# snayfach/MicrobeCensus

Measured on AMD Instinct MI355X. Metric: reads/sec searched vs marker DB + AGS abs-error, 150 bp @ 1/2/4/8 GPU, higher is better.
Workload: dtype u8/int32

## Files before the change

microbecensus_amd/csrc/k_translate_seg.h:

```cpp
#pragma once
#include "mc_hip_common.h"

#define MC_TS_THREADS 64
#define MC_TS_WAVES (MC_TS_THREADS / 64)
#define MC_TS_READS (MC_TS_THREADS / 6)
#define MC_TS_NLNF(FP) ((FP) + 2 > 24 ? (FP) + 2 : 24)
#define MC_TS_STRIDE(FP) (((((FP) + 76 + 3) >> 2) | 1) << 2)
#define MC_TS_STAGE(L) ((((MC_TS_READS * (L)) > MC_TS_WAVES * 1488 ? (MC_TS_READS * (L)) : MC_TS_WAVES * 1488) + 15) & ~15)

struct McSegWaveLds { unsigned long long best[64]; uint32_t pre[66]; uint32_t pre2[66]; uint32_t bq[64]; uint16_t off[64]; uint8_t n[64]; };
static_assert(sizeof(McHsp) == 48 && sizeof(McGapTask) % 4 == 0, "k_eval_seeds copies its staging buffers as 16- and 4-byte words");
static_assert(sizeof(McSegWaveLds) == 1488, "MC_TS_STAGE reserves 1488 bytes per wave");
#ifdef MC_EXP_TIMING
__device__ unsigned long long g_ts_acc[12], g_ts_cnt[12];
#define MC_TS_TICK(k) do { const unsigned long long now_ = __builtin_readcyclecounter(); if (lane == 0) { ts_acc_[tcat_] += now_ - tlast_; ts_acc_[12 + tcat_] += 1; } tlast_ = now_; tcat_ = (k); } while (0)
#define MC_TS_BEGIN(k) __shared__ unsigned long long ts_acc_[24]; if (lane < 24) ts_acc_[lane] = 0; mc_wave_sync(); unsigned long long tlast_ = __builtin_readcyclecounter(); int tcat_ = (k)
#define MC_TS_PARAMS , unsigned long long &tlast_, int &tcat_, unsigned long long *ts_acc_
#define MC_TS_ARGS , tlast_, tcat_, ts_acc_
#define MC_TS_END do { mc_wave_sync(); if (lane < 12) { atomicAdd(&g_ts_acc[lane], ts_acc_[lane]); atomicAdd(&g_ts_cnt[lane], ts_acc_[12 + lane]); } } while (0)
#else
#define MC_TS_TICK(k) do { } while (0)
#define MC_TS_BEGIN(k) do { } while (0)
#define MC_TS_PARAMS
#define MC_TS_ARGS
#define MC_TS_END do { } while (0)
#endif
#define MC_SEG_KEY_ONE 0xBFF0000000000000ull

__device__ __forceinline__ unsigned long long mc_seg_key(double x)
{
    const unsigned long long u = (unsigned long long)__double_as_longlong(x);
    return (u >> 63) ? ~u : (u | 0x8000000000000000ull);
}

__device__ __forceinline__ void mc_seg_wave(const double *lnf, const int32_t *fx, const uint64_t *__restrict__ segtab, uint8_t *prot, int n, bool act, const McSegWS ws, McSegWaveLds *WL,
                                         const uint8_t *lds0, int lane MC_TS_PARAMS)
{
    const int W = (n <= 11) ? 8 : 12;
    MC_TS_TICK(0);
    enum { POP = 0, SCAN = 1, WAIT = 2, DONE = 3 };
    int st = (act && W <= n) ? POP : DONE;
    McBits192 Flo, Fhi, lo, nhi, mk;
    mc_bits_clear(Flo); mc_bits_clear(Fhi); mc_bits_clear(lo); mc_bits_clear(nhi); mc_bits_clear(mk);
    if (st != DONE) {
        mc_seg_window_flags_rg(fx, prot, n, W, Flo, Fhi);
        if (!(Flo.a | Flo.b | Flo.c)) st = DONE;
    }
    int sp = 1, base = 0, m = 0, i = 0, lowlim = 0, loi = 0, hii = 0;
    bool any = false;
    if (st != DONE) { ws.stk[0] = 0; ws.stk[1] = (int16_t)n; }
    const unsigned long long ltmask = (1ull << lane) - 1;
    for (;;) {
        MC_TS_TICK(1);
        while (st == POP || st == SCAN) {
            if (st == POP) {
                if (sp == 0) { st = DONE; break; }
                sp--;
                base = ws.stk[2 * sp]; m = ws.stk[2 * sp + 1];
                if (W > m) continue;
                lo = mc_seg_flags_of(Flo, base, m, W);
                i = mc_bits_next(lo, 0);
                if (i >= m) continue;
                nhi = mc_bits_andnot(mc_bits_low(m), mc_seg_flags_of(Fhi, base, m, W));
                lowlim = 0; st = SCAN;
            }
            loi = mc_bits_prev(nhi, i) + 1; if (loi < lowlim) loi = lowlim;
            hii = mc_bits_next(nhi, i) - 1; if (hii > m - 1) hii = m - 1;
            st = WAIT;
        }
        const unsigned long long req = __ballot(st == WAIT);
        MC_TS_TICK(2);
        if (req == 0) break;
        const int nreq = __popcll(req);
        const int myr = __popcll(req & ltmask);
        const int myn = hii - loi + 1;
        if (st == WAIT) {
            WL->off[myr] = (uint16_t)((prot + base + loi) - lds0);
            WL->n[myr] = (uint8_t)myn;
            WL->best[myr] = MC_SEG_KEY_ONE; WL->bq[myr] = 0xFFFFFFFFu;
        }
        mc_wave_sync();
#define MC_SEG_CJ(j, sh) (((((j) >> (sh)) * (((j) >> (sh)) + 1)) << (sh)) / 2 + ((j) & ((1 << (sh)) - 1)) * (((j) >> (sh)) + 1))
        int sh0 = 3, sh1 = 3;
        {
            int K = 0, j0 = 0;
            if (lane < nreq) { const int nn = WL->n[lane], minlen = (nn - 100 > 1) ? nn - 100 : 1; K = nn - minlen; j0 = nn - 15 > 0 ? (nn - 15 < K ? nn - 15 : K) : 0; }
            uint32_t s0 = 0, s1 = 0;
#pragma unroll
            for (int sh = 2; sh >= 0; sh--) {
                const uint32_t c1 = (uint32_t)MC_SEG_CJ(j0, sh), c0 = (uint32_t)MC_SEG_CJ(K, sh) - c1;
                const uint32_t t0 = (uint32_t)__builtin_amdgcn_readlane((int)mc_wave_scan_add(c0), 63), t1 = (uint32_t)__builtin_amdgcn_readlane((int)mc_wave_scan_add(c1), 63);
                if (t0 <= 64) sh0 = sh;
                if (t1 <= 64) sh1 = sh;
            }
            {
                const uint32_t c1 = sh1 == 0 ? (uint32_t)MC_SEG_CJ(j0, 0) : sh1 == 1 ? (uint32_t)MC_SEG_CJ(j0, 1) : sh1 == 2 ? (uint32_t)MC_SEG_CJ(j0, 2) : (uint32_t)MC_SEG_CJ(j0, 3);
                const uint32_t cj0 = sh0 == 0 ? (uint32_t)MC_SEG_CJ(j0, 0) : sh0 == 1 ? (uint32_t)MC_SEG_CJ(j0, 1) : sh0 == 2 ? (uint32_t)MC_SEG_CJ(j0, 2) : (uint32_t)MC_SEG_CJ(j0, 3);
                const uint32_t ck = sh0 == 0 ? (uint32_t)MC_SEG_CJ(K, 0) : sh0 == 1 ? (uint32_t)MC_SEG_CJ(K, 1) : sh0 == 2 ? (uint32_t)MC_SEG_CJ(K, 2) : (uint32_t)MC_SEG_CJ(K, 3);
                s0 = mc_wave_scan_add(ck - cj0); s1 = mc_wave_scan_add(c1);
            }
            if (lane == 0) { WL->pre[0] = 0; WL->pre2[0] = 0; }
            WL->pre[lane + 1] = s0; WL->pre2[lane + 1] = s1;
        }
        mc_wave_sync();
        for (int cls = 0; cls < 2; cls++) {
        const uint32_t *pre = cls ? WL->pre2 : WL->pre;
        const uint32_t total = pre[nreq];
        const int sh = cls ? sh1 : sh0, R = 1 << sh;
        for (uint32_t p0 = 0; p0 < total; p0 += 64) {
            MC_TS_TICK(3 + cls);
            const uint32_t p = p0 + (uint32_t)lane;
            const bool ok = p < total;
            int r = 0;
            for (int stp = 32; stp > 0; stp >>= 1) { const int k = r + stp; if (k < nreq && p >= pre[k]) r = k; }
            if (!ok) r = 0;
            const int nn = WL->n[r];
            int x = (int)(p - pre[r]);
            if (cls == 0) { const int minlen = (nn - 100 > 1) ? nn - 100 : 1, K = nn - minlen, j0 = nn - 15 > 0 ? (nn - 15 < K ? nn - 15 : K) : 0; x += MC_SEG_CJ(j0, sh); }
            int A = (int)((sqrtf(1.0f + 8.0f * (float)x / (float)R) - 1.0f) * 0.5f);
            while ((((A + 1) * (A + 2)) << sh) / 2 <= x) A++;
            while (((A * (A + 1)) << sh) / 2 > x) A--;
            const int rem = x - ((A * (A + 1)) << sh) / 2, B = rem / (A + 1), run = rem - B * (A + 1);
            const int j = (A << sh) + B, wfirst = run << sh, wlast = (wfirst + R - 1 < j) ? wfirst + R - 1 : j;
            const uint8_t *s = lds0 + WL->off[r];
            const int len = nn - j;
            const uint32_t qbase = (uint32_t)(j * (j + 1) / 2);
            unsigned long long key = MC_SEG_KEY_ONE;
            uint32_t kq = 0xFFFFFFFFu;
            if (ok) {
                if (cls == 0) {
                    McRhState rg; rg.clo = 0; rg.chi = 0; rg.hist = 0;
                    for (int k = 0; k < len; k++) mc_rh_add(rg, s[wfirst + k]);
                    const int cnt = wlast - wfirst + 1;
                    uint64_t svs[8];
#pragma unroll
                    for (int t = 0; t < 8; t++) {
                        svs[t] = rg.hist | ((uint64_t)len << 60);
                        if (t + 1 < cnt) { mc_rh_remove(rg, s[wfirst + t]); mc_rh_add(rg, s[wfirst + t + len]); }
                    }
#pragma unroll
                    for (int t0 = 0; t0 < 8; t0 += 4) {
                        if (t0 && R <= 4) break;
                        ulonglong2 ea[4], eb[4];
#pragma unroll
                        for (int t = 0; t < 4; t++) {
                            uint32_t h1, h2;
                            mc_segtab_slots(svs[t0 + t], h1, h2);
                            const bool in = t0 + t < cnt;
                            ea[t] = ((const ulonglong2 *)segtab)[in ? h1 : 0u]; eb[t] = ((const ulonglong2 *)segtab)[in ? h2 : 0u];
                        }
#pragma unroll
                        for (int t = 0; t < 4; t++)
                            if (t0 + t < cnt) {
                                const unsigned long long pk = ea[t].x == svs[t0 + t] ? ea[t].y : eb[t].y;
                                if (pk < key) { key = pk; kq = qbase + (uint32_t)(wfirst + t0 + t); }
                            }
                    }
                } else {
                    mc_seg_comp_rg(s + wfirst, len, ws.comp);
                    mc_seg_state(ws.comp, ws.sv);
                    for (int w0 = wfirst;; w0++) {
                        const unsigned long long k2 = mc_seg_key(mc_seg_getprob(lnf, ws.sv, len));
                        if (k2 < key) { key = k2; kq = qbase + (uint32_t)w0; }
                        if (w0 == wlast) break;
                        mc_seg_shift(ws.comp, ws.sv, s[w0], s[w0 + len]);
                    }
                }
            }
            MC_TS_TICK(5);
            const bool cand = ok && key < MC_SEG_KEY_ONE;
            const unsigned long long old = WL->best[r];
            mc_wave_sync();
            if (cand) atomicMin(&WL->best[r], key);
            mc_wave_sync();
            const unsigned long long nb = WL->best[r];
            if (ok && nb != old) WL->bq[r] = 0xFFFFFFFFu;
            mc_wave_sync();
            if (cand && key == nb) atomicMin(&WL->bq[r], kq);
            mc_wave_sync();
        }
        }
#undef MC_SEG_CJ
        MC_TS_TICK(6);
        if (st == WAIT) {
            const uint32_t q = WL->bq[myr];
            int lend = 0, rend = myn - 1;
            if (q != 0xFFFFFFFFu) {
                int j = (int)((sqrtf((float)(8u * q + 1u)) - 1.0f) * 0.5f);
                while ((uint32_t)((j + 1) * (j + 2) / 2) <= q) j++;
                while ((uint32_t)(j * (j + 1) / 2) > q) j--;
                const int len = myn - j, w0 = (int)q - j * (j + 1) / 2;
                lend = w0; rend = len + w0 - 1;
            }
            const int leftend = loi + lend, rightend = hii - (myn - rend - 1);
            if (i < leftend) {
                const int l2 = loi, r2 = leftend - 1;
// ... 33 lines not shown
            w[k >> 2] |= ((a0 | a1 | a2) < 0 ? (uint32_t)MC_INV : aa) << (8 * (k & 3));
        }
        *(uint32_t *)(prot + i) = w[0];
        *(uint32_t *)(prot + i + 4) = w[1];
    }
    for (; i < n; i++) {
        const int a0 = mc_nt_code(p[s * (3 * i)], set, perm), a1 = mc_nt_code(p[s * (3 * i + 1)], set, perm), a2 = mc_nt_code(p[s * (3 * i + 2)], set, perm);
        const uint8_t aa = cod[(16 * a0 + 4 * a1 + a2) & 63];
        prot[i] = (a0 | a1 | a2) < 0 ? (uint8_t)MC_INV : aa;
    }
    return n;
}

template <bool STAGED>
__global__ void __attribute__((amdgpu_waves_per_eu(4, 4))) __launch_bounds__(MC_TS_THREADS) k_translate_seg(const McTables *__restrict__ T, const uint8_t *__restrict__ reads, int L,
                                                       int64_t nreads, uint8_t *__restrict__ frames, int FP, const uint64_t *__restrict__ segtab)
{
    extern __shared__ __attribute__((aligned(16))) uint8_t smem[];
    const int tid = threadIdx.x;
    const int64_t r0 = (int64_t)blockIdx.x * MC_TS_READS;
    const int nr = (int)((nreads - r0) < MC_TS_READS ? (nreads - r0) : MC_TS_READS);
    const int rbytes = nr * L;
    const int stride = MC_TS_STRIDE(FP);
    __shared__ int32_t fxs[64];
#ifdef MC_EXP_TIMING
    const int lane = mc_lane();
#endif
    MC_TS_BEGIN(8);
    uint8_t *sreads = smem;
    const int nlnf = MC_TS_NLNF(FP);
    double *lnf = (double *)(smem + (STAGED ? MC_TS_STAGE(L) : MC_TS_STAGE(0)));
    uint8_t *rows = (uint8_t *)(lnf + nlnf);
    __shared__ __attribute__((aligned(4))) uint8_t cod[64];
    if (tid < 64) fxs[tid] = T->seg_dout[tid];
    if (tid < 16) ((uint32_t *)cod)[tid] = ((const uint32_t *)T->codon)[tid];
    for (int i = tid; i < nlnf; i += MC_TS_THREADS) lnf[i] = T->lnfac[i];
    if (STAGED) {
        const uint8_t *src = reads + r0 * L;
        const int head = (int)((4 - ((uintptr_t)src & 3)) & 3), nhead = head < rbytes ? head : rbytes;
        if (tid < nhead) sreads[tid] = src[tid];
        const int nw = (rbytes - nhead) >> 2;
        if (nhead == 0) for (int i = tid; i < nw; i += MC_TS_THREADS) ((uint32_t *)sreads)[i] = ((const uint32_t *)src)[i];
        else for (int i = tid; i < nw; i += MC_TS_THREADS) { const uint32_t w = ((const uint32_t *)(src + nhead))[i]; uint8_t *d = sreads + nhead + 4 * i; d[0] = (uint8_t)w; d[1] = (uint8_t)(w >> 8); d[2] = (uint8_t)(w >> 16); d[3] = (uint8_t)(w >> 24); }
        for (int i = nhead + 4 * nw + tid; i < rbytes; i += MC_TS_THREADS) sreads[i] = src[i];
    }
    __syncthreads();
    MC_TS_TICK(9);
    const int lr = tid / 6, f = tid - lr * 6;
    uint8_t *prot = rows + (size_t)tid * stride;
    int n = 0;
    if (lr < nr) n = mc_translate_frame_lds(cod, STAGED ? sreads + lr * L : reads + (r0 + lr) * L, L, f, prot);
    __syncthreads();
    {
        McSegWS ws; ws.comp = prot + FP; ws.sv = prot + FP + 20; ws.stk = (int16_t *)(prot + FP + 44);
        mc_seg_wave(lnf, fxs, segtab, prot, n, lr < nr, ws, (McSegWaveLds *)smem + (tid >> 6), rows, mc_lane() MC_TS_ARGS);
        if (lr < nr) for (int i = n; i < FP; i++) prot[i] = MC_INV;
    }
    __syncthreads();
    {
        uint32_t *dst = (uint32_t *)(frames + r0 * 6 * FP);
        const int total = nr * 6 * FP / 4, fpw = FP / 4;
        for (int i = tid; i < total; i += MC_TS_THREADS) { const int row = i / fpw, col = i - row * fpw; dst[i] = *(const uint32_t *)(rows + (size_t)row * stride + 4 * col); }
    }
    MC_TS_TICK(0);
    MC_TS_END;
}
```

microbecensus_amd/csrc/mc_core.h:

```cpp
#pragma once
#include <stdint.h>

#if defined(__HIPCC__)
#include <hip/hip_runtime.h>
#define MC_HD __host__ __device__ __forceinline__
#define MC_HDN __host__ __device__
#else
#define MC_HD inline
#define MC_HDN inline
struct uint4 { uint32_t x, y, z, w; };
inline uint4 make_uint4(uint32_t x, uint32_t y, uint32_t z, uint32_t w) { uint4 v; v.x = x; v.y = y; v.z = z; v.w = w; return v; }
#endif

#define MC_NBUCKET 1000000
#define MC_INV 20
#define MC_INVGRP 10
#define MC_MAXAA 170
#define MC_SMAX 4096
#define MC_MAX_M8 500
#define MC_LNFAC_N 400

#define MC_GAP_OPEN 11
#define MC_GAP_EXT 1
#define MC_SEG_FXBITS 24
// ... 375 lines not shown
MC_HD void mc_segtab_slots(uint64_t k, uint32_t &h1, uint32_t &h2)
{
    const uint32_t lo = (uint32_t)k, hi = (uint32_t)(k >> 32);
    uint32_t x = (lo ^ (hi << 7) ^ (((hi >> 28) * 0x924000u) & 0x04444000u)) * 0xBA1BF32Fu;
    x ^= x >> 15;
    h1 = x >> (32 - MC_SEGTAB_LOG2);
    h2 = (x >> 6) & (MC_SEGTAB_SLOTS - 1);
}
MC_HD uint64_t mc_segtab_lookup(const uint64_t *tab, uint64_t hist, int len)
{
    const uint64_t k = hist | ((uint64_t)len << 60);
    uint32_t h1, h2;
    mc_segtab_slots(k, h1, h2);
    if (tab[2 * h1] == k) return tab[2 * h1 + 1];
    return tab[2 * h2] == k ? tab[2 * h2 + 1] : 0;
}

MC_HD void mc_seg_trim_rg(const double *lnfac, const uint8_t *s, int n, int *leftend, int *rightend)
{
    int lend = 0, rend = n - 1;
    double minprob = 1.0;
    McRgState st0; st0.clo = 0; st0.chi = 0; st0.sv = 0;
    for (int k = 0; k < n; k++) mc_rg_add(st0, s[k]);
    for (int len = n; len > 1; len--) {
        McRgState st = st0;
        for (int i = 0;; i++) {
            const double prob = mc_rg_getprob(lnfac, st.sv, len);
            if (prob < minprob) { minprob = prob; lend = i; rend = len + i - 1; }
            if (i + 1 + len > n) break;
            mc_rg_remove(st, s[i]); mc_rg_add(st, s[i + len]);
// ... 242 lines not shown
    int sp = 1;
    ws.stk[0] = 0; ws.stk[1] = (int16_t)n;
    bool any = false;
    while (sp > 0) {
        sp--;
        const int base = ws.stk[2 * sp], m = ws.stk[2 * sp + 1];
        const uint8_t *s = prot + base;
        if (W > m) continue;
        const McBits192 lo = mc_seg_flags_of(Flo, base, m, W), hi = mc_seg_flags_of(Fhi, base, m, W);
        const McBits192 nhi = mc_bits_andnot(mc_bits_low(m), hi);
        int lowlim = 0;
        for (int i = mc_bits_next(lo, 0); i < m; i = mc_bits_next(lo, i + 1)) {
            int loi = mc_bits_prev(nhi, i) + 1; if (loi < lowlim) loi = lowlim;
            int hii = mc_bits_next(nhi, i) - 1; if (hii > m - 1) hii = m - 1;
            int leftend = loi, rightend = hii;
            if (rightend - leftend + 1 <= 15) mc_seg_trim_rg(lnfac, s + leftend, rightend - leftend + 1, &leftend, &rightend);
            else mc_seg_trim_ws(lnfac, s + leftend, rightend - leftend + 1, &leftend, &rightend, ws);
            if (i < leftend) {
                const int lend = loi, rend = leftend - 1;
                if (sp < 8) { ws.stk[2 * sp] = (int16_t)(base + lend); ws.stk[2 * sp + 1] = (int16_t)(rend - lend + 1); sp++; }
            }
            mk = mc_bits_or(mk, mc_bits_range(base + leftend, base + rightend));
            any = true;
            i = (hii < rightend) ? hii : rightend;
            lowlim = i + 1;
        }
    }
    if (any) for (int i = 0; i < n; i++) if (mc_bits_test(mk, i)) prot[i] = MC_INV;
}

// ... 682 lines not shown
```

microbecensus_amd/csrc/mc_hip.hip:

```cpp
#include "mc_hip_common.h"
#include "k_translate_seg.h"
#include "k_enumerate.h"
#include "k_eval_seeds.h"
#include "k_gapped.h"
#include "k_order.h"
#include "k_finish.h"
#include "k_grid.h"
#include "k_simulate.h"
#include "k_community.h"
#include "k_varlen.h"
#include "k_bootstrap.h"

#include <map>

struct McCtx {
    hipStream_t stream = nullptr, side = nullptr, side2 = nullptr;
    hipEvent_t ev[8] = {}, ev_fork = nullptr, ev_join = nullptr, ev_join2 = nullptr;
    int64_t cap_reads = 0; int pool_len = 0;
    uint32_t cap_tasks = 0, cap_gaps = 0, cap_hsps = 0, cap_rows = 0;
    uint8_t *d_frames = nullptr, *d_frames_base = nullptr;
    unsigned long long *d_stats = nullptr;
    McSeedTask *d_tasks = nullptr; McGapTask *d_gaps = nullptr; McHsp *d_hsps = nullptr, *d_v = nullptr, *d_tmp = nullptr;
    uint64_t *d_k64 = nullptr, *d_hkeys = nullptr, *d_hplace = nullptr, *d_places = nullptr; uint32_t *d_idx = nullptr, *d_idxo = nullptr, *d_heads = nullptr, *d_scan = nullptr, *d_gsz = nullptr, *d_nv = nullptr; uint32_t *d_ghist = nullptr;
    uint32_t *d_counters = nullptr;
// ... 4 lines not shown
    const uint8_t *reads = nullptr; int64_t n = 0, first_read_id = 0;
    uint32_t ntasks = 0, ngaps = 0, gpad = 0, nh = 0, nh_all = 0, nheads = 0, nrows = 0, nbest = 0, nsegs = 0;
    bool busy = false;
};

struct mc_handle {
    McHostIndex H;
    std::vector<int32_t> fam;
    int nfam = 0, device = 0;
    uint8_t *d_res = nullptr, *d_res_base = nullptr; uint32_t *d_off = nullptr, *d_bstart = nullptr, *d_post = nullptr; unsigned long long *d_post8 = nullptr; uint16_t *d_keys = nullptr; int32_t *d_fam = nullptr;
    McTables *d_T = nullptr; McClassPars *d_P = nullptr;
    McTables hT; McClassPars hP;
    int read_len = 0, FP = 0; bool run_set = false;
    uint32_t *d_bitmap = nullptr;
    McBucketRec *d_rec = nullptr;
    uint32_t *d_filt = nullptr, *d_wild = nullptr, *d_pair = nullptr; uint64_t *d_segtab = nullptr; unsigned long long *d_rt = nullptr;
    bool fast_enum = false;
    bool count_traffic = false;
    int pipe_nout = 0;
    bool keep_rows = true;
    bool best_only = false;
    bool rows_stay = false;
    float train_ms[3] = {0, 0, 0};
    float comm_ms[2] = {0, 0};
    int64_t train_bases = 0;
    float boot_ms = 0;
    uint8_t *stage_pin[2] = {}, *stage_dev[2] = {}; size_t stage_bytes = 0; hipStream_t copy_stream = nullptr;
    int64_t nreads = 0, cap_own = 0;
    uint8_t *d_reads = nullptr;
    const uint8_t *reads_dev = nullptr;
    McCtx ctx;
// ... 32 lines not shown
{
    void *ptrs[] = {c.d_frames_base, c.d_tasks, c.d_gaps, c.d_hsps, c.d_v, c.d_tmp, c.d_k64, c.d_hkeys, c.d_hplace, c.d_places, c.d_idx, c.d_idxo, c.d_heads, c.d_scan, c.d_gsz, c.d_nv, c.d_ghist, c.d_counters, c.d_rows,
                    c.d_nrow, c.d_rowoff, c.d_best, c.d_bestof, c.d_low, c.d_cand, c.d_gws_full, c.d_retry, c.d_retry2, c.d_gtab, c.d_gleader, c.d_fout, c.d_stats};
    for (void *p : ptrs) if (p) (void)hipFree(p);
    for (void *p : {(void *)c.h_c, (void *)c.h_stats, (void *)c.h_best}) if (p) (void)hipHostFree(p);
    for (auto &e : c.ev) if (e) (void)hipEventDestroy(e);
    for (hipEvent_t e : {c.ev_fork, c.ev_join, c.ev_join2}) if (e) (void)hipEventDestroy(e);
    if (c.stream) (void)hipStreamDestroy(c.stream);
    c = McCtx();
}

extern "C" void mc_close(mc_handle *h)
{
    if (!h) return;
    (void)hipSetDevice(h->device);
    void *ptrs[] = {h->d_res_base, h->d_off, h->d_bstart, h->d_post, h->d_post8, h->d_keys, h->d_fam, h->d_T, h->d_P, h->d_reads, h->d_bitmap, h->d_rec, h->d_filt, h->d_wild, h->d_pair, h->d_rt, h->d_segtab};
    for (void *p : ptrs) if (p) (void)hipFree(p);
    ctx_free(h->ctx);
    for (int k = 0; k < 2; k++) { if (h->stage_pin[k]) (void)hipHostFree(h->stage_pin[k]); if (h->stage_dev[k]) (void)hipFree(h->stage_dev[k]); }
    if (h->copy_stream) (void)hipStreamDestroy(h->copy_stream);
    for (hipStream_t q : {h->side, h->side2}) if (q) (void)hipStreamDestroy(q);
    if (h->rows_stream) { (void)hipStreamSynchronize(h->rows_stream); (void)hipStreamDestroy(h->rows_stream); }
    if (h->ev_rows) (void)hipEventDestroy(h->ev_rows);
    for (mc_row *p : h->pin_slot) if (p) (void)hipHostFree(p);
    delete h;
}

struct McUploader {
    static constexpr size_t CH = (size_t)8 << 20;
    uint8_t *pin[2] = {nullptr, nullptr}; hipEvent_t ev[2] = {nullptr, nullptr}; hipStream_t st = nullptr; int k = 0; bool used[2] = {false, false};
    int init()
// ... 211 lines not shown
    HIPCK(hipSetDevice(h->device));
    double t0 = mc_now();
    mc_fill_tables(h->hT, h->H, read_len, loge_thr);
    MC_OT("set_run: tables", t0);
    if (mc_seg_fx_verify(h->hT, nullptr) != 0) { g_err = "internal: the fixed-point SEG tests disagree with the reference arithmetic"; return -1; }
    MC_OT("set_run: seg_fx_verify", t0);
    memset(&h->hP, 0, sizeof h->hP);
    h->hP.nfam = h->nfam; h->hP.read_len = read_len;
    for (int f = 0; f < h->nfam; f++) { h->hP.min_cov[f] = min_cov[f]; h->hP.min_score[f] = min_score[f]; h->hP.max_aaid[f] = max_aaid[f]; h->hP.aln_stat[f] = aln_stat[f]; }
    HIPCK(hipMemcpy(h->d_T, &h->hT, sizeof(McTables), hipMemcpyHostToDevice));
    if (!h->d_segtab) {
        std::vector<uint64_t> tab;
        mc_build_segtab(h->hT.lnfac, tab);
        if (dalloc(&h->d_segtab, tab.size())) return -1;
        HIPCK(hipMemcpy(h->d_segtab, tab.data(), tab.size() * 8, hipMemcpyHostToDevice));
    }
    HIPCK(hipMemcpy(h->d_P, &h->hP, sizeof(McClassPars), hipMemcpyHostToDevice));
    const int newFP = ((read_len / 3 + 2) + 3) & ~3;
    if (newFP != h->FP || read_len != h->read_len) h->ctx.cap_reads = 0;
    h->read_len = read_len; h->FP = newFP; h->run_set = true;
    MC_OT("set_run: segtab, uploads", t0);
    return 0;
}

static void best_materialize(mc_handle *h);
static int ensure_capacity(mc_handle *h, McCtx &c, int64_t nreads)
{
    if (nreads <= c.cap_reads && h->read_len <= c.pool_len) return 0;
    if (h->best_from == &c) best_materialize(h);
    double t0 = mc_now();
// ... 45 lines not shown
    return 0;
}

static float ev_ms(hipEvent_t a, hipEvent_t b) { float ms = 0; (void)hipEventElapsedTime(&ms, a, b); return ms; }

static int stage_wait(McCtx &c) { HIPCK(hipStreamSynchronize(c.stream)); return 0; }
static int counters_to_host(McCtx &c) { HIPCK(hipMemcpyAsync(c.h_c, c.d_counters, sizeof(uint32_t) * C_N, hipMemcpyDeviceToHost, c.stream)); return 0; }

#ifdef MC_EXP_TIMING
static int exp_timing_dump(McCtx &c, char stage)
{
    if (stage == 'a') {
        HIPCK(hipStreamSynchronize(c.stream));
        unsigned long long acc[12], cnt[12];
        HIPCK(hipMemcpyFromSymbol(acc, HIP_SYMBOL(g_ts_acc), sizeof acc)); HIPCK(hipMemcpyFromSymbol(cnt, HIP_SYMBOL(g_ts_cnt), sizeof cnt));
        const char *nm[12] = {"flags", "advance", "numbering", "class-0 rounds", "class-1 rounds", "reduction", "owners", "mask", "staging", "translation", "write-out", ""};
        const double waves = (double)((c.n + MC_TS_READS - 1) / MC_TS_READS) * MC_TS_WAVES;
        for (int k = 0; k < 11; k++) fprintf(stderr, "ts-timing %-15s %9.1f cycles/wave  %8.2f entries/wave  total %8.1f Mcycles\n", nm[k], (double)acc[k] / waves, (double)cnt[k] / waves, acc[k] / 1e6);
        unsigned long long z[12] = {0, 0, 0, 0, 0, 0, 0, 0, 0, 0, 0, 0};
        HIPCK(hipMemcpyToSymbol(HIP_SYMBOL(g_ts_acc), z, sizeof z)); HIPCK(hipMemcpyToSymbol(HIP_SYMBOL(g_ts_cnt), z, sizeof z));
    } else {
        HIPCK(hipStreamSynchronize(c.stream)); HIPCK(hipStreamSynchronize(c.side));
        unsigned long long acc[8], cnt[8];
        HIPCK(hipMemcpyFromSymbol(acc, HIP_SYMBOL(g_fh_acc), sizeof acc)); HIPCK(hipMemcpyFromSymbol(cnt, HIP_SYMBOL(g_fh_cnt), sizeof cnt));
        {
            unsigned long long fr[8];
            HIPCK(hipMemcpyFromSymbol(fr, HIP_SYMBOL(g_fr_acc), sizeof fr));
            const char *fn[7] = {"groups", "items", "std::sort", "threshold, keys", "heap sort", "rows", "classification"};
            for (int k = 0; k < 7; k++) fprintf(stderr, "fr-timing %-17s total %9.1f Mcycles (thread wall time, summed)\n", fn[k], fr[k] / 1e6);
            unsigned long long z8[8] = {0, 0, 0, 0, 0, 0, 0, 0};
            HIPCK(hipMemcpyToSymbol(HIP_SYMBOL(g_fr_acc), z8, sizeof z8));
            HIPCK(hipMemcpyFromSymbol(fr, HIP_SYMBOL(g_fr_acc2), sizeof fr));
            const char *gn[8] = {"-", "sort by frame", "sort by start, stable", "choice", "sum statistics", "copies", "groups (count)", "groups linked (count)"};
// ... 43 lines not shown
    HIPCK(hipMemsetAsync(c.d_counters, 0, sizeof(uint32_t) * C_N, st));
    HIPCK(hipMemsetAsync(c.d_stats, 0, sizeof(unsigned long long) * S_N, st));
    if (h->best_only) HIPCK(hipMemsetAsync(c.d_cand, 0, (size_t)n, st));
    HIPCK(hipMemsetAsync(c.d_low, 0, (size_t)n, st));
    HIPCK(hipEventRecord(c.ev[0], st));
    const int64_t threads = n * 6;
    const size_t lds_rest = (size_t)MC_TS_NLNF(FP) * 8 + (size_t)MC_TS_THREADS * MC_TS_STRIDE(FP);
    const size_t lds_staged = (size_t)MC_TS_STAGE(L) + lds_rest, lds_direct = (size_t)MC_TS_STAGE(0) + lds_rest;
    static const int ts_force = getenv("MC_TS_STAGED") ? atoi(getenv("MC_TS_STAGED")) : -1;
    const size_t cu_lds = 160 * 1024 - 1024;
    const bool staged = ts_force >= 0 ? ts_force != 0 : cu_lds / lds_staged >= cu_lds / lds_direct;
    const size_t lds = staged ? lds_staged : lds_direct;
    const unsigned ts_blocks = (unsigned)((n + MC_TS_READS - 1) / MC_TS_READS);
    if (staged) {
        if (lds > 48 * 1024) HIPCK(hipFuncSetAttribute((const void *)k_translate_seg<true>, hipFuncAttributeMaxDynamicSharedMemorySize, (int)lds));
        k_translate_seg<true><<<dim3(ts_blocks), dim3(MC_TS_THREADS), lds, st>>>(h->d_T, c.reads, L, n, c.d_frames, FP, h->d_segtab);
    } else {
        if (lds > 48 * 1024) HIPCK(hipFuncSetAttribute((const void *)k_translate_seg<false>, hipFuncAttributeMaxDynamicSharedMemorySize, (int)lds));
        k_translate_seg<false><<<dim3(ts_blocks), dim3(MC_TS_THREADS), lds, st>>>(h->d_T, c.reads, L, n, c.d_frames, FP, h->d_segtab);
    }
    HIPCK(hipEventRecord(c.ev[1], st));
    if (exp_timing_dump(c, 'a')) return -1;
    if (h->fast_enum) {
        const bool enq = !h->count_traffic;
        const size_t per_wave = enq ? MC_ENQ_WAVE_LDS(FP, L) : sizeof(McEnWave) + MC_EN_WAVE_LDS(FP, L);
        int waves = 0, bpc = 1;
        {
            static const int shapes_q[][2] = {{8, 2}, {4, 4}, {16, 1}, {12, 1}, {4, 3}, {8, 1}, {4, 2}, {4, 1}};
            static const int shapes_c[][2] = {{12, 2}, {8, 3}, {4, 6}, {4, 5}, {16, 1}, {8, 2}, {4, 4}, {12, 1}, {4, 3}, {8, 1}, {4, 2}, {4, 1}};
            if (enq) { for (const auto &sh : shapes_q) if (!waves && (size_t)sh[1] * (64 + sh[0] * per_wave) <= 160 * 1024) { waves = sh[0]; bpc = sh[1]; } }
            else for (const auto &sh : shapes_c) if (!waves && (size_t)sh[1] * (64 + sh[0] * per_wave) <= 160 * 1024) { waves = sh[0]; bpc = sh[1]; }
        }
        if (!waves) { g_err = "reads too long for the seed kernel's LDS layout"; return -1; }
        const size_t lds2 = 64 + waves * per_wave;
// ... 1318 lines not shown
```

microbecensus_amd/csrc/mc_index.h:

```cpp
#pragma once
#include <sys/stat.h>
#include <unistd.h>
#include "mc_core.h"
#include <math.h>
#include <stdio.h>
#include <stdlib.h>
#include <string.h>
#include <string>
#include <vector>
#include <algorithm>

struct McHostIndex {
    std::vector<std::string> names;
    std::vector<uint8_t> res_code;
    std::vector<uint8_t> res;
    std::vector<uint32_t> off, bstart, post;
    std::vector<uint16_t> keys;
    std::vector<uint32_t> bitmap;
    std::vector<McBucketRec> rec;
    std::vector<uint32_t> filt;
    std::vector<uint32_t> wild;
    std::vector<uint32_t> pair;
    std::vector<unsigned long long> rt;
    uint32_t rt_mask;
// ... 542 lines not shown
                }
                npairs++;
            }
        }
        void go(uint64_t sv, int nparts, int t, int maxpart)
        {
            emit(sv, t);
            if (nparts == 15) return;
            for (int p = 1; p <= maxpart && t + p <= 15; p++) go(sv | ((uint64_t)p << (4 * nparts)), nparts + 1, t + p, p);
        }
    } rec{lnfac, tab, npairs};
    rec.go(0, 0, 0, 15);
    (void)npairs;
}

inline void mc_fill_tables(McTables &T, const McHostIndex &X, int read_len, double loge_thr)
{
    static const int8_t B62[20][20] = {
        {4, -1, -2, -2, 0, -1, -1, 0, -2, -1, -1, -1, -1, -2, -1, 1, 0, -3, -2, 0}, {-1, 5, 0, -2, -3, 1, 0, -2, 0, -3, -2, 2, -1, -3, -2, -1, -1, -3, -2, -3},
        {-2, 0, 6, 1, -3, 0, 0, 0, 1, -3, -3, 0, -2, -3, -2, 1, 0, -4, -2, -3}, {-2, -2, 1, 6, -3, 0, 2, -1, -1, -3, -4, -1, -3, -3, -1, 0, -1, -4, -3, -3},
        {0, -3, -3, -3, 9, -3, -4, -3, -3, -1, -1, -3, -1, -2, -3, -1, -1, -2, -2, -1}, {-1, 1, 0, 0, -3, 5, 2, -2, 0, -3, -2, 1, 0, -3, -1, 0, -1, -2, -1, -2},
        {-1, 0, 0, 2, -4, 2, 5, -2, 0, -3, -3, 1, -2, -3, -1, 0, -1, -3, -2, -2}, {0, -2, 0, -1, -3, -2, -2, 6, -2, -4, -4, -2, -3, -3, -2, 0, -2, -2, -3, -3},
        {-2, 0, 1, -1, -3, 0, 0, -2, 8, -3, -3, -1, -2, -1, -2, -1, -2, -2, 2, -3}, {-1, -3, -3, -3, -1, -3, -3, -4, -3, 4, 2, -3, 1, 0, -3, -2, -1, -3, -1, 3},
        {-1, -2, -3, -4, -1, -2, -3, -4, -3, 2, 4, -2, 2, 0, -3, -2, -1, -2, -1, 1}, {-1, 2, 0, -1, -3, 1, 1, -2, -1, -3, -2, 5, -1, -3, -1, 0, -1, -3, -2, -2},
        {-1, -1, -2, -3, -1, 0, -2, -3, -2, 1, 2, -1, 5, 0, -2, -1, -1, -1, -1, 1}, {-2, -3, -3, -3, -2, -3, -3, -3, -1, 0, 0, -3, 0, 6, -4, -2, -2, 1, 3, -1},
        {-1, -2, -2, -1, -3, -1, -1, -2, -2, -3, -3, -1, -2, -4, 7, -1, -1, -4, -3, -2}, {1, -1, 1, 0, -1, 0, 0, 0, -1, -2, -2, 0, -1, -2, -1, 4, 1, -3, -2, -2},
        {0, -1, 0, -1, -1, -1, -1, -2, -2, -1, -1, -1, -1, -2, -1, 1, 5, -2, -2, 0}, {-3, -3, -4, -4, -2, -2, -3, -2, -2, -3, -2, -3, -1, 1, -4, -3, -2, 11, 2, -3},
        {-2, -2, -2, -3, -2, -1, -2, -3, 2, -1, -1, -2, -1, 3, -3, -2, -2, 2, 7, -1}, {0, -3, -3, -3, -1, -2, -2, -3, -3, 3, 1, -2, 1, -1, -2, -2, 0, -3, -1, 4}};
    static const char *aa = "FFLLSSSSYY..CC.WLLLLPPPPHHQQRRRRIIIMTTTTNNKKSSRRVVVVAAAADDEEGGGG";
    const double LN2 = 0.6931471805599453;
// ... 44 lines not shown
```

Measured before the change: 63.74 million.

## Add hashed composition lookup table for SEG windows of length 16-32

After: 64.30 million (median of 6 runs). Within noise of the previous version (+0.9%).

```diff
diff --git a/microbecensus_amd/csrc/k_translate_seg.h b/microbecensus_amd/csrc/k_translate_seg.h
--- a/microbecensus_amd/csrc/k_translate_seg.h
+++ b/microbecensus_amd/csrc/k_translate_seg.h
@@ -33,8 +33,8 @@
     return (u >> 63) ? ~u : (u | 0x8000000000000000ull);
 }
 
-__device__ __forceinline__ void mc_seg_wave(const double *lnf, const int32_t *fx, const uint64_t *__restrict__ segtab, uint8_t *prot, int n, bool act, const McSegWS ws, McSegWaveLds *WL,
-                                         const uint8_t *lds0, int lane MC_TS_PARAMS)
+__device__ __forceinline__ void mc_seg_wave(const double *lnf, int32_t *fx, const uint64_t *__restrict__ segtab, const uint64_t *__restrict__ segtab2, uint8_t *prot, int n, bool act, const McSegWS ws,
+                                         McSegWaveLds *WL, const uint8_t *lds0, int lane MC_TS_PARAMS)
 {
     const int W = (n <= 11) ? 8 : 12;
     MC_TS_TICK(0);
@@ -50,6 +50,8 @@
     bool any = false;
     if (st != DONE) { ws.stk[0] = 0; ws.stk[1] = (int16_t)n; }
     const unsigned long long ltmask = (1ull << lane) - 1;
+    uint64_t *Z = (uint64_t *)fx;
+    bool zin = false;
     for (;;) {
         MC_TS_TICK(1);
         while (st == POP || st == SCAN) {
@@ -75,54 +77,74 @@
         const int myr = __popcll(req & ltmask);
         const int myn = hii - loi + 1;
         if (st == WAIT) {
-            WL->off[myr] = (uint16_t)((prot + base + loi) - lds0);
+            int ninv = 0;
+            if (myn > 15)
+                for (int k = 0; k < myn && ninv <= MC_SEGTAB2_MAXLACK; k += 8) {
+#pragma unroll
+                    for (int q = 0; q < 8; q++) ninv += (k + q < myn) & (prot[base + loi + (k + q < myn ? k + q : myn - 1)] >= 20);
+                }
+            WL->off[myr] = (uint16_t)(((prot + base + loi) - lds0) | (myn > 15 && ninv <= MC_SEGTAB2_MAXLACK ? 0x8000 : 0));
             WL->n[myr] = (uint8_t)myn;
             WL->best[myr] = MC_SEG_KEY_ONE; WL->bq[myr] = 0xFFFFFFFFu;
         }
         mc_wave_sync();
 #define MC_SEG_CJ(j, sh) (((((j) >> (sh)) * (((j) >> (sh)) + 1)) << (sh)) / 2 + ((j) & ((1 << (sh)) - 1)) * (((j) >> (sh)) + 1))
-        int sh0 = 3, sh1 = 3;
+#define MC_SEG_CJS(j, sh) ((sh) == 0 ? (uint32_t)MC_SEG_CJ(j, 0) : (sh) == 1 ? (uint32_t)MC_SEG_CJ(j, 1) : (sh) == 2 ? (uint32_t)MC_SEG_CJ(j, 2) : (uint32_t)MC_SEG_CJ(j, 3))
+#define MC_SEG_JT(nn, cov, j0) ((cov) ? ((nn) - MC_SEGTAB2_MAXLEN > 0 ? ((nn) - MC_SEGTAB2_MAXLEN < (j0) ? (nn) - MC_SEGTAB2_MAXLEN : (j0)) : 0) : (j0))
+        int sh0 = 3, sh1 = 3, sh2 = 3;
         {
-            int K = 0, j0 = 0;
-            if (lane < nreq) { const int nn = WL->n[lane], minlen = (nn - 100 > 1) ? nn - 100 : 1; K = nn - minlen; j0 = nn - 15 > 0 ? (nn - 15 < K ? nn - 15 : K) : 0; }
-            uint32_t s0 = 0, s1 = 0;
+            int K = 0, j0 = 0, jT = 0;
+            if (lane < nreq) {
+                const int nn = WL->n[lane], minlen = (nn - 100 > 1) ? nn - 100 : 1;
+                K = nn - minlen; j0 = nn - 15 > 0 ? (nn - 15 < K ? nn - 15 : K) : 0; jT = MC_SEG_JT(nn, WL->off[lane] >> 15, j0);
+            }
+            uint32_t s0 = 0, s12 = 0;
 #pragma unroll
             for (int sh = 2; sh >= 0; sh--) {
-                const uint32_t c1 = (uint32_t)MC_SEG_CJ(j0, sh), c0 = (uint32_t)MC_SEG_CJ(K, sh) - c1;
-                const uint32_t t0 = (uint32_t)__builtin_amdgcn_readlane((int)mc_wave_scan_add(c0), 63), t1 = (uint32_t)__builtin_amdgcn_readlane((int)mc_wave_scan_add(c1), 63);
+                const uint32_t cT = (uint32_t)MC_SEG_CJ(jT, sh), c1 = (uint32_t)MC_SEG_CJ(j0, sh) - cT, c0 = (uint32_t)MC_SEG_CJ(K, sh) - (uint32_t)MC_SEG_CJ(j0, sh);
+                const uint32_t c12 = (c1 < 1023u ? c1 : 1023u) | ((cT < 1023u ? cT : 1023u) << 16);
+                const uint32_t t0 = (uint32_t)__builtin_amdgcn_readlane((int)mc_wave_scan_add(c0), 63), t12 = (uint32_t)__builtin_amdgcn_readlane((int)mc_wave_scan_add(c12), 63);
                 if (t0 <= 64) sh0 = sh;
-                if (t1 <= 64) sh1 = sh;
+                if ((t12 & 0xFFFFu) <= 64) sh1 = sh;
+                if ((t12 >> 16) <= 64) sh2 = sh;
             }
             {
-                const uint32_t c1 = sh1 == 0 ? (uint32_t)MC_SEG_CJ(j0, 0) : sh1 == 1 ? (uint32_t)MC_SEG_CJ(j0, 1) : sh1 == 2 ? (uint32_t)MC_SEG_CJ(j0, 2) : (uint32_t)MC_SEG_CJ(j0, 3);
-                const uint32_t cj0 = sh0 == 0 ? (uint32_t)MC_SEG_CJ(j0, 0) : sh0 == 1 ? (uint32_t)MC_SEG_CJ(j0, 1) : sh0 == 2 ? (uint32_t)MC_SEG_CJ(j0, 2) : (uint32_t)MC_SEG_CJ(j0, 3);
-                const uint32_t ck = sh0 == 0 ? (uint32_t)MC_SEG_CJ(K, 0) : sh0 == 1 ? (uint32_t)MC_SEG_CJ(K, 1) : sh0 == 2 ? (uint32_t)MC_SEG_CJ(K, 2) : (uint32_t)MC_SEG_CJ(K, 3);
-                s0 = mc_wave_scan_add(ck - cj0); s1 = mc_wave_scan_add(c1);
+                const uint32_t cT = MC_SEG_CJS(jT, sh2), c1 = MC_SEG_CJS(j0, sh1) - MC_SEG_CJS(jT, sh1), c0 = MC_SEG_CJS(K, sh0) - MC_SEG_CJS(j0, sh0);
+                s0 = mc_wave_scan_add(c0); s12 = mc_wave_scan_add(c1 | (cT << 16));
             }
             if (lane == 0) { WL->pre[0] = 0; WL->pre2[0] = 0; }
-            WL->pre[lane + 1] = s0; WL->pre2[lane + 1] = s1;
+            WL->pre[lane + 1] = s0; WL->pre2[lane + 1] = s12;
         }
         mc_wave_sync();
-        for (int cls = 0; cls < 2; cls++) {
-        const uint32_t *pre = cls ? WL->pre2 : WL->pre;
-        const uint32_t total = pre[nreq];
-        const int sh = cls ? sh1 : sh0, R = 1 << sh;
+        if (!zin && (WL->pre2[nreq] & 0xFFFFu) != 0) {
+            if (lane <= MC_SEGTAB2_MAXLEN) Z[lane] = segtab2[lane];
+            zin = true;
+            mc_wave_sync();
+        }
+        for (int cls = 0; cls < 3; cls++) {
+#define MC_SEG_PRE(k) (cls == 0 ? WL->pre[k] : cls == 1 ? (WL->pre2[k] & 0xFFFFu) : (WL->pre2[k] >> 16))
+        const uint32_t total = MC_SEG_PRE(nreq);
+        const int sh = cls == 0 ? sh0 : cls == 1 ? sh1 : sh2, R = 1 << sh;
         for (uint32_t p0 = 0; p0 < total; p0 += 64) {
-            MC_TS_TICK(3 + cls);
+            MC_TS_TICK(cls == 2 ? 11 : 3 + cls);
             const uint32_t p = p0 + (uint32_t)lane;
             const bool ok = p < total;
             int r = 0;
-            for (int stp = 32; stp > 0; stp >>= 1) { const int k = r + stp; if (k < nreq && p >= pre[k]) r = k; }
+            for (int stp = 32; stp > 0; stp >>= 1) { const int k = r + stp; if (k < nreq && p >= MC_SEG_PRE(k)) r = k; }
             if (!ok) r = 0;
             const int nn = WL->n[r];
-            int x = (int)(p - pre[r]);
-            if (cls == 0) { const int minlen = (nn - 100 > 1) ? nn - 100 : 1, K = nn - minlen, j0 = nn - 15 > 0 ? (nn - 15 < K ? nn - 15 : K) : 0; x += MC_SEG_CJ(j0, sh); }
+            const uint32_t offr = WL->off[r];
+            int x = (int)(p - MC_SEG_PRE(r));
+            if (cls < 2) {
+                const int minlen = (nn - 100 > 1) ? nn - 100 : 1, K = nn - minlen, j0 = nn - 15 > 0 ? (nn - 15 < K ? nn - 15 : K) : 0, jT = MC_SEG_JT(nn, offr >> 15, j0);
+                x += (int)MC_SEG_CJS(cls == 0 ? j0 : jT, sh);
+            }
             int A = (int)((sqrtf(1.0f + 8.0f * (float)x / (float)R) - 1.0f) * 0.5f);
             while ((((A + 1) * (A + 2)) << sh) / 2 <= x) A++;
             while (((A * (A + 1)) << sh) / 2 > x) A--;
             const int rem = x - ((A * (A + 1)) << sh) / 2, B = rem / (A + 1), run = rem - B * (A + 1);
             const int j = (A << sh) + B, wfirst = run << sh, wlast = (wfirst + R - 1 < j) ? wfirst + R - 1 : j;
-            const uint8_t *s = lds0 + WL->off[r];
+            const uint8_t *s = lds0 + (offr & 0x7FFFu);
             const int len = nn - j;
             const uint32_t qbase = (uint32_t)(j * (j + 1) / 2);
             unsigned long long key = MC_SEG_KEY_ONE;
@@ -153,6 +175,35 @@
                         for (int t = 0; t < 4; t++)
                             if (t0 + t < cnt) {
                                 const unsigned long long pk = ea[t].x == svs[t0 + t] ? ea[t].y : eb[t].y;
+                                if (pk < key) { key = pk; kq = qbase + (uint32_t)(wfirst + t0 + t); }
+                            }
+                    }
+                } else if (cls == 1) {
+                    McRkState rk;
+                    mc_rk_init(rk, s + wfirst, len, Z);
+                    const int cnt = wlast - wfirst + 1;
+                    const ulonglong2 *slots = (const ulonglong2 *)(segtab2 + MC_SEGTAB2_HEAD);
+#pragma unroll
+                    for (int t0 = 0; t0 < 8; t0 += 2) {
+                        if (t0 >= R) break;
+                        uint64_t kws[2];
+#pragma unroll
+                        for (int t = 0; t < 2; t++) {
+                            kws[t] = mc_segtab2_key(rk.acc, len);
+                            if (t0 + t + 1 < cnt) { mc_rk_remove(rk, s[wfirst + t0 + t], Z); mc_rk_add(rk, s[wfirst + t0 + t + len], Z); }
+                        }
+                        ulonglong2 ea[2], eb[2];
+#pragma unroll
+                        for (int t = 0; t < 2; t++) {
+                            uint32_t h1, h2;
+                            mc_segtab2_slots(kws[t], h1, h2);
+                            const bool in = t0 + t < cnt;
+                            ea[t] = slots[in ? h1 : 0u]; eb[t] = slots[in ? h2 : 0u];
+                        }
+#pragma unroll
+                        for (int t = 0; t < 2; t++)
+                            if (t0 + t < cnt) {
+                                const unsigned long long pk = ea[t].x == kws[t] ? ea[t].y : eb[t].y;
                                 if (pk < key) { key = pk; kq = qbase + (uint32_t)(wfirst + t0 + t); }
                             }
                     }
@@ -180,6 +231,9 @@
             mc_wave_sync();
         }
         }
+#undef MC_SEG_PRE
+#undef MC_SEG_JT
+#undef MC_SEG_CJS
 #undef MC_SEG_CJ
         MC_TS_TICK(6);
         if (st == WAIT) {
@@ -243,7 +297,7 @@
 
 template <bool STAGED>
 __global__ void __attribute__((amdgpu_waves_per_eu(4, 4))) __launch_bounds__(MC_TS_THREADS) k_translate_seg(const McTables *__restrict__ T, const uint8_t *__restrict__ reads, int L,
-                                                       int64_t nreads, uint8_t *__restrict__ frames, int FP, const uint64_t *__restrict__ segtab)
+                                                       int64_t nreads, uint8_t *__restrict__ frames, int FP, const uint64_t *__restrict__ segtab, const uint64_t *__restrict__ segtab2)
 {
     extern __shared__ __attribute__((aligned(16))) uint8_t smem[];
     const int tid = threadIdx.x;
@@ -251,7 +305,9 @@
     const int nr = (int)((nreads - r0) < MC_TS_READS ? (nreads - r0) : MC_TS_READS);
     const int rbytes = nr * L;
     const int stride = MC_TS_STRIDE(FP);
-    __shared__ int32_t fxs[64];
+    __shared__ __attribute__((aligned(8))) uint32_t stat[80];
+    int32_t *fxs = (int32_t *)stat;
+    static_assert((MC_SEGTAB2_MAXLEN + 1) * 8 <= sizeof(uint32_t) * 80, "Z[0..32] lies where the entropy and codon tables lay");
 #ifdef MC_EXP_TIMING
     const int lane = mc_lane();
 #endif
@@ -260,7 +316,7 @@
     const int nlnf = MC_TS_NLNF(FP);
     double *lnf = (double *)(smem + (STAGED ? MC_TS_STAGE(L) : MC_TS_STAGE(0)));
     uint8_t *rows = (uint8_t *)(lnf + nlnf);
-    __shared__ __attribute__((aligned(4))) uint8_t cod[64];
+    uint8_t *cod = (uint8_t *)(stat + 64);
     if (tid < 64) fxs[tid] = T->seg_dout[tid];
     if (tid < 16) ((uint32_t *)cod)[tid] = ((const uint32_t *)T->codon)[tid];
     for (int i = tid; i < nlnf; i += MC_TS_THREADS) lnf[i] = T->lnfac[i];
@@ -282,7 +338,7 @@
     __syncthreads();
     {
         McSegWS ws; ws.comp = prot + FP; ws.sv = prot + FP + 20; ws.stk = (int16_t *)(prot + FP + 44);
-        mc_seg_wave(lnf, fxs, segtab, prot, n, lr < nr, ws, (McSegWaveLds *)smem + (tid >> 6), rows, mc_lane() MC_TS_ARGS);
+        mc_seg_wave(lnf, fxs, segtab, segtab2, prot, n, lr < nr, ws, (McSegWaveLds *)smem + (tid >> 6), rows, mc_lane() MC_TS_ARGS);
         if (lr < nr) for (int i = n; i < FP; i++) prot[i] = MC_INV;
     }
     __syncthreads();
diff --git a/microbecensus_amd/csrc/mc_core.h b/microbecensus_amd/csrc/mc_core.h
--- a/microbecensus_amd/csrc/mc_core.h
+++ b/microbecensus_amd/csrc/mc_core.h
@@ -413,6 +413,63 @@
     mc_segtab_slots(k, h1, h2);
     if (tab[2 * h1] == k) return tab[2 * h1 + 1];
     return tab[2 * h2] == k ? tab[2 * h2 + 1] : 0;
+}
+#define MC_SEGTAB2_MINLEN 16
+#define MC_SEGTAB2_MAXLEN 32
+#define MC_SEGTAB2_MAXLACK 2
+#define MC_SEGTAB2_HEAD 34
+#define MC_SEGTAB2_LOG2 18
+#define MC_SEGTAB2_SLOTS (1u << MC_SEGTAB2_LOG2)
+struct McRkState { uint64_t c0, c1; uint32_t c2; uint64_t acc; };
+MC_HD int mc_rk_count(const McRkState &st, int r)
+{
+    const int sh = (r & 7) * 8;
+    return (int)(((r < 8 ? st.c0 : r < 16 ? st.c1 : (uint64_t)st.c2) >> sh) & 255);
+}
+MC_HD void mc_rk_bump(McRkState &st, int r, bool up)
+{
+    const uint64_t inc = 1ull << ((r & 7) * 8), d = up ? inc : 0 - inc;
+    if (r < 8) st.c0 += d; else if (r < 16) st.c1 += d; else st.c2 += (uint32_t)d;
+}
+MC_HD void mc_rk_add(McRkState &st, int r, const uint64_t *Z)
+{
+    if (r >= 20) return;
+    const int x = mc_rk_count(st, r);
+    st.acc += Z[x + 1] - Z[x];
+    mc_rk_bump(st, r, true);
+}
+MC_HD void mc_rk_remove(McRkState &st, int r, const uint64_t *Z)
+{
+    if (r >= 20) return;
+    const int x = mc_rk_count(st, r);
+    st.acc += Z[x - 1] - Z[x];
+    mc_rk_bump(st, r, false);
+}
+MC_HD void mc_rk_init(McRkState &st, const uint8_t *s, int n, const uint64_t *Z)
+{
+    st.c0 = 0; st.c1 = 0; st.c2 = 0; st.acc = 0;
+    for (int i = 0; i < n; i++) { const int r = s[i]; if (r < 20) mc_rk_bump(st, r, true); }
+    uint64_t a = 0, b = 0;
+#pragma unroll 1
+    for (int k = 0; k < 8; k += 2) { a += Z[(st.c0 >> (8 * k)) & 255] + Z[(st.c1 >> (8 * k)) & 255]; b += Z[(st.c0 >> (8 * k + 8)) & 255] + Z[(st.c1 >> (8 * k + 8)) & 255]; }
+    for (int k = 0; k < 4; k += 2) { a += Z[(st.c2 >> (8 * k)) & 255]; b += Z[(st.c2 >> (8 * k + 8)) & 255]; }
+    st.acc = a + b;
+}
+MC_HD uint64_t mc_segtab2_key(uint64_t acc, int len) { return (acc & ((1ull << 58) - 1)) | ((uint64_t)len << 58); }
+MC_HD void mc_segtab2_slots(uint64_t k, uint32_t &h1, uint32_t &h2)
+{
+    const uint32_t len = (uint32_t)(k >> 58);
+    h1 = ((uint32_t)k + len * 0x9E3779B1u) & (MC_SEGTAB2_SLOTS - 1);
+    h2 = ((uint32_t)(k >> MC_SEGTAB2_LOG2) + len * 0x85EBCA6Bu) & (MC_SEGTAB2_SLOTS - 1);
+    if (h2 == h1) h2 ^= 1u;
+}
+MC_HD uint64_t mc_segtab2_lookup(const uint64_t *tab, uint64_t acc, int len)
+{
+    const uint64_t k = mc_segtab2_key(acc, len), *slots = tab + MC_SEGTAB2_HEAD;
+    uint32_t h1, h2;
+    mc_segtab2_slots(k, h1, h2);
+    if (slots[2 * h1] == k) return slots[2 * h1 + 1];
+    return slots[2 * h2] == k ? slots[2 * h2 + 1] : 0;
 }
 
 MC_HD void mc_seg_trim_rg(const double *lnfac, const uint8_t *s, int n, int *leftend, int *rightend)
@@ -685,6 +742,9 @@
             int loi = mc_bits_prev(nhi, i) + 1; if (loi < lowlim) loi = lowlim;
             int hii = mc_bits_next(nhi, i) - 1; if (hii > m - 1) hii = m - 1;
             int leftend = loi, rightend = hii;
+#ifdef MC_SEG_CENSUS
+            MC_SEG_CENSUS(s + leftend, rightend - leftend + 1);
+#endif
             if (rightend - leftend + 1 <= 15) mc_seg_trim_rg(lnfac, s + leftend, rightend - leftend + 1, &leftend, &rightend);
             else mc_seg_trim_ws(lnfac, s + leftend, rightend - leftend + 1, &leftend, &rightend, ws);
             if (i < leftend) {
diff --git a/microbecensus_amd/csrc/mc_hip.hip b/microbecensus_amd/csrc/mc_hip.hip
--- a/microbecensus_amd/csrc/mc_hip.hip
+++ b/microbecensus_amd/csrc/mc_hip.hip
@@ -42,7 +42,7 @@
     int read_len = 0, FP = 0; bool run_set = false;
     uint32_t *d_bitmap = nullptr;
     McBucketRec *d_rec = nullptr;
-    uint32_t *d_filt = nullptr, *d_wild = nullptr, *d_pair = nullptr; uint64_t *d_segtab = nullptr; unsigned long long *d_rt = nullptr;
+    uint32_t *d_filt = nullptr, *d_wild = nullptr, *d_pair = nullptr; uint64_t *d_segtab = nullptr, *d_segtab2 = nullptr; unsigned long long *d_rt = nullptr;
     bool fast_enum = false;
     bool count_traffic = false;
     int pipe_nout = 0;
@@ -105,7 +105,7 @@
 {
     if (!h) return;
     (void)hipSetDevice(h->device);
-    void *ptrs[] = {h->d_res_base, h->d_off, h->d_bstart, h->d_post, h->d_post8, h->d_keys, h->d_fam, h->d_T, h->d_P, h->d_reads, h->d_bitmap, h->d_rec, h->d_filt, h->d_wild, h->d_pair, h->d_rt, h->d_segtab};
+    void *ptrs[] = {h->d_res_base, h->d_off, h->d_bstart, h->d_post, h->d_post8, h->d_keys, h->d_fam, h->d_T, h->d_P, h->d_reads, h->d_bitmap, h->d_rec, h->d_filt, h->d_wild, h->d_pair, h->d_rt, h->d_segtab, h->d_segtab2};
     for (void *p : ptrs) if (p) (void)hipFree(p);
     ctx_free(h->ctx);
     for (int k = 0; k < 2; k++) { if (h->stage_pin[k]) (void)hipHostFree(h->stage_pin[k]); if (h->stage_dev[k]) (void)hipFree(h->stage_dev[k]); }
@@ -347,6 +347,12 @@
         mc_build_segtab(h->hT.lnfac, tab);
         if (dalloc(&h->d_segtab, tab.size())) return -1;
         HIPCK(hipMemcpy(h->d_segtab, tab.data(), tab.size() * 8, hipMemcpyHostToDevice));
+    }
+    if (!h->d_segtab2) {
+        std::vector<uint64_t> tab;
+        mc_build_segtab2(h->hT.lnfac, tab);
+        if (dalloc(&h->d_segtab2, tab.size())) return -1;
+        HIPCK(hipMemcpy(h->d_segtab2, tab.data(), tab.size() * 8, hipMemcpyHostToDevice));
     }
     HIPCK(hipMemcpy(h->d_P, &h->hP, sizeof(McClassPars), hipMemcpyHostToDevice));
     const int newFP = ((read_len / 3 + 2) + 3) & ~3;
@@ -422,9 +428,9 @@
         HIPCK(hipStreamSynchronize(c.stream));
         unsigned long long acc[12], cnt[12];
         HIPCK(hipMemcpyFromSymbol(acc, HIP_SYMBOL(g_ts_acc), sizeof acc)); HIPCK(hipMemcpyFromSymbol(cnt, HIP_SYMBOL(g_ts_cnt), sizeof cnt));
-        const char *nm[12] = {"flags", "advance", "numbering", "class-0 rounds", "class-1 rounds", "reduction", "owners", "mask", "staging", "translation", "write-out", ""};
+        const char *nm[12] = {"flags", "advance", "numbering", "class-0 rounds", "class-1 rounds", "reduction", "owners", "mask", "staging", "translation", "write-out", "class-2 rounds"};
         const double waves = (double)((c.n + MC_TS_READS - 1) / MC_TS_READS) * MC_TS_WAVES;
-        for (int k = 0; k < 11; k++) fprintf(stderr, "ts-timing %-15s %9.1f cycles/wave  %8.2f entries/wave  total %8.1f Mcycles\n", nm[k], (double)acc[k] / waves, (double)cnt[k] / waves, acc[k] / 1e6);
+        for (int k = 0; k < 12; k++) fprintf(stderr, "ts-timing %-15s %9.1f cycles/wave  %8.2f entries/wave  total %8.1f Mcycles\n", nm[k], (double)acc[k] / waves, (double)cnt[k] / waves, acc[k] / 1e6);
         unsigned long long z[12] = {0, 0, 0, 0, 0, 0, 0, 0, 0, 0, 0, 0};
         HIPCK(hipMemcpyToSymbol(HIP_SYMBOL(g_ts_acc), z, sizeof z)); HIPCK(hipMemcpyToSymbol(HIP_SYMBOL(g_ts_cnt), z, sizeof z));
     } else {
@@ -498,10 +504,10 @@
     const unsigned ts_blocks = (unsigned)((n + MC_TS_READS - 1) / MC_TS_READS);
     if (staged) {
         if (lds > 48 * 1024) HIPCK(hipFuncSetAttribute((const void *)k_translate_seg<true>, hipFuncAttributeMaxDynamicSharedMemorySize, (int)lds));
-        k_translate_seg<true><<<dim3(ts_blocks), dim3(MC_TS_THREADS), lds, st>>>(h->d_T, c.reads, L, n, c.d_frames, FP, h->d_segtab);
+        k_translate_seg<true><<<dim3(ts_blocks), dim3(MC_TS_THREADS), lds, st>>>(h->d_T, c.reads, L, n, c.d_frames, FP, h->d_segtab, h->d_segtab2);
     } else {
         if (lds > 48 * 1024) HIPCK(hipFuncSetAttribute((const void *)k_translate_seg<false>, hipFuncAttributeMaxDynamicSharedMemorySize, (int)lds));
-        k_translate_seg<false><<<dim3(ts_blocks), dim3(MC_TS_THREADS), lds, st>>>(h->d_T, c.reads, L, n, c.d_frames, FP, h->d_segtab);
+        k_translate_seg<false><<<dim3(ts_blocks), dim3(MC_TS_THREADS), lds, st>>>(h->d_T, c.reads, L, n, c.d_frames, FP, h->d_segtab, h->d_segtab2);
     }
     HIPCK(hipEventRecord(c.ev[1], st));
     if (exp_timing_dump(c, 'a')) return -1;
diff --git a/microbecensus_amd/csrc/mc_index.h b/microbecensus_amd/csrc/mc_index.h
--- a/microbecensus_amd/csrc/mc_index.h
+++ b/microbecensus_amd/csrc/mc_index.h
@@ -580,6 +580,53 @@
     (void)npairs;
 }
 
+inline void mc_segtab2_terms(uint64_t *Z )
+{
+    uint64_t x = 0x5E6C0DE5A17AB1E5ull;
+    Z[0] = 0;
+    for (int c = 1; c <= MC_SEGTAB2_MAXLEN; c++) { x += 0x9E3779B97F4A7C15ull; uint64_t z = x; z = (z ^ (z >> 30)) * 0xBF58476D1CE4E5B9ull; z = (z ^ (z >> 27)) * 0x94D049BB133111EBull; Z[c] = z ^ (z >> 31); }
+}
+inline size_t mc_build_segtab2(const double *lnfac, std::vector<uint64_t> &tab)
+{
+    tab.assign((size_t)MC_SEGTAB2_HEAD + (size_t)MC_SEGTAB2_SLOTS * 2, 0);
+    mc_segtab2_terms(tab.data());
+    std::vector<uint64_t> seen;
+    struct Rec {
+        const double *lnfac; std::vector<uint64_t> &tab; std::vector<uint64_t> &seen; uint8_t sv[24];
+        void emit(int nparts, int len)
+        {
+            const uint64_t *Z = tab.data();
+            uint64_t *slots = tab.data() + MC_SEGTAB2_HEAD;
+            uint64_t acc = 0;
+            for (int i = 0; i < nparts; i++) acc += Z[sv[i]];
+            sv[nparts] = 0;
+            uint64_t ck = mc_segtab2_key(acc, len), cv = mc_seg_prob_key(mc_seg_getprob(lnfac, sv, len));
+            seen.push_back(ck);
+            uint32_t at = 0xFFFFFFFFu;
+            for (int kick = 0;; kick++) {
+                if (kick >= 512) { fprintf(stderr, "mc_build_segtab2: no placement\n"); abort(); }
+                uint32_t h1, h2;
+                mc_segtab2_slots(ck, h1, h2);
+                const uint32_t h = (at == h1) ? h2 : h1;
+                std::swap(ck, slots[2 * h]); std::swap(cv, slots[2 * h + 1]);
+                at = h;
+                if (ck == 0) break;
+            }
+        }
+        void go(int nparts, int left, int maxpart, int len)
+        {
+            if (left == 0) { emit(nparts, len); return; }
+            if (nparts == 20) return;
+            for (int p = 1; p <= maxpart && p <= left; p++) { sv[nparts] = (uint8_t)p; go(nparts + 1, left - p, p, len); }
+        }
+    } rec{lnfac, tab, seen, {0}};
+    for (int len = MC_SEGTAB2_MINLEN; len <= MC_SEGTAB2_MAXLEN; len++)
+        for (int lack = 0; lack <= MC_SEGTAB2_MAXLACK; lack++) rec.go(0, len - lack, len - lack, len);
+    std::sort(seen.begin(), seen.end());
+    for (size_t i = 1; i < seen.size(); i++) if (seen[i] == seen[i - 1]) { fprintf(stderr, "mc_build_segtab2: two pairs share a key word\n"); abort(); }
+    return seen.size();
+}
+
 inline void mc_fill_tables(McTables &T, const McHostIndex &X, int read_len, double loge_thr)
 {
     static const int8_t B62[20][20] = {
```
